# TensorSpeech/TensorFlowASR

Hardware: AMD Instinct MI355X
Metric: audio-hours/sec (train step) Conformer-M RNN-T (higher is better)
Workload: dtype bf16; 1 GPU; Conformer-M transducer full train step (fwd+RNN-T loss+bwd+Adam), LibriSpeech-shaped 16 kHz utterances, 32/GPU, padding=batch, SpecAugment on, dropout 0.1; global_batch=32, parallelism=dp1, params=32461288

## Files before the change

### include/tfasr_hip.h

```cpp
#ifndef TFASR_HIP_H_
#define TFASR_HIP_H_

#include <stddef.h>
#include <stdint.h>

#ifdef __cplusplus
extern "C" {
#endif

#define TFASR_ABI_VERSION 44

typedef enum {
  TFASR_STATUS_SUCCESS = 0,
  TFASR_STATUS_INVALID_VALUE = 1,
  TFASR_STATUS_EXECUTION_FAILED = 2,
  TFASR_STATUS_UNSUPPORTED = 3
} tfasr_status_t;

typedef enum { TFASR_F32 = 0, TFASR_BF16 = 1 } tfasr_dtype_t;

const char* tfasr_status_string(int status);
int tfasr_abi_version(void);
size_t tfasr_launch_count(void);

// ... 161 lines not shown

int tfasr_relattn_softmax_fwd(const void* content, const void* pos, const int32_t* lengths, void* probs, int B, int H,
                              int T, int ldc, int ldp, int use_mask, int dtype, void* stream);
int tfasr_relattn_softmax_bwd(const void* probs, const void* dprobs, const int32_t* lengths, void* dcontent, void* dpos,
                              int B, int H, int T, int ldc, int ldp, int use_mask, int dtype, void* stream);
int tfasr_relattn_softmax_fwd_streaming(const void* content, const void* pos, const int32_t* lengths, void* probs, int B, int H,
                                        int T, int ldc, int ldp, int use_mask, int chunk_size, int history_size, int dtype,
                                        void* stream);

int tfasr_relattn_fused_fwd(const void* qkv, const float* ubias, const float* vbias, const void* pext,
                            const int32_t* lengths, void* out, float* lse, int B, int H, int T, int dh, float scale,
                            int use_mask, int chunk, int hist, int dtype, void* stream);

int tfasr_relattn_fused_bwd_q3(const void* qkv, const float* ubias, const float* vbias, const void* pext, const int32_t* lengths,
                               const void* o, const void* dout, const float* lse, void* dq, long lddq, float* du, float* dv, void* ds,
                               float* dvec, float* dpext, void* qu, void* qv, int B, int H, int T, int dh, int lds, float scale, int use_mask,
                               int chunk, int hist, int dtype, void* stream);
int tfasr_relattn_dpext(const void* ds, const void* qv, const int32_t* lengths, float* dpext, int B, int H, int T, int dh, int lds,
                        int use_mask, int dtype, void* stream);
int tfasr_relattn_fused_bwd_k(const void* qkv, const void* qu, const void* qv, const void* pext, const int32_t* lengths,
                              const void* dout, const float* lse, const float* dvec, void* dqkv, int B, int H, int T, int dh,
                              float scale, int use_mask, int chunk, int hist, int dtype, void* stream);

int tfasr_lstm_step_fwd(const void* xg, long xg_stride_b, const float* hr, const void* h_prev, long hprev_stride_b,
                        const float* c_prev, long cprev_stride_b, const int32_t* lengths, int t, void* gates,
                        long gates_stride_b, float* c_out, long c_stride_b, void* h_out, long h_stride_b, void* y_out,
                        long y_stride_b, int B, int P, int dtype, void* stream);
int tfasr_lstm_step_bwd(const void* dy, long dy_stride_b, const float* dhr, float* dh_carry, float* dc_carry,
                        const void* gates, long gates_stride_b, const float* c_t, long c_stride_b, const float* c_prev,
                        long cprev_stride_b, const int32_t* lengths, int t, void* dz, long dz_stride_b, int B, int P,
                        int dtype, void* stream);

int tfasr_lstm_set_persist(int mode);
int tfasr_lstm_seq_fwd(const void* xg, const void* rk, const void* h0, long h0_stride_b, const float* c0, long c0_stride_b,
                       const int32_t* lengths, void* gates, float* cseq, void* hseq, void* yseq, float* hr, int B, int U1, int P,
                       int dtype, void* stream);
int tfasr_lstm_seq_bwd(const void* dy, const void* rk, const void* gates, const float* cseq, const int32_t* lengths, void* dz,
                       float* dh_carry, float* dc_carry, float* dhr, int B, int U1, int P, int dtype, void* stream);
int tfasr_lstm_seq_fwd_range(const void* xg, const void* rk, const void* h0, long h0_stride_b, const float* c0, long c0_stride_b,
                             const int32_t* lengths, void* gates, float* cseq, void* hseq, void* yseq, float* hr, int B, int U1, int P,
                             int dtype, int t0, int t1, void* stream);
int tfasr_lstm_seq_bwd_range(const void* dy, const void* rk, const void* gates, const float* cseq, const int32_t* lengths, void* dz,
                             float* dh_carry, float* dc_carry, float* dhr, int B, int U1, int P, int dtype, int t0, int t1, void* stream);
size_t tfasr_lstm_persist_sync_bytes(void);
int tfasr_lstm_persist_fwd(const void* xg, const void* rk, const void* h0, long h0_stride_b, const float* c0, long c0_stride_b,
                           const int32_t* lengths, void* gates, float* cseq, void* hseq, void* yseq, int B, int U1, int P, int dtype,
// ... 256 lines not shown
```

### tensorflowasr_amd/csrc/attn_fused.hip

```cpp
#include "common.h"
#ifdef TFASR_ATTN_TIMING
__device__ long long g_attn_timing[8 * 8192];
#define ATT_TICK(k) { const long long t_ = __builtin_readcyclecounter(); ph[k] += t_ - tp; tp = t_; }
#else
#define ATT_TICK(k)
#endif
#include <algorithm>
#include <stdlib.h>

typedef __attribute__((ext_vector_type(4))) short short4_t;

namespace {

#define LDS_PTR(p) ((__attribute__((address_space(3))) void*)(p))
#define GLB_PTR(p) ((const __attribute__((address_space(1))) void*)(p))

constexpr int DH = 64, BI = 64, BJ = 64, WIN = 128;
constexpr int SK_BYTES = BJ * DH * 2, SV_BYTES = BJ * DH * 2, SP_BYTES = WIN * DH * 2;
__device__ __forceinline__ int key_d(int row) { return (row & 3) | (((row >> 3) & 1) << 2); }
__device__ __forceinline__ int key_t64(int k) { return (((k >> 1) & 1) | (((k >> 3) & 1) << 1)) << 1; }

__device__ __forceinline__ void glds16_asm(const void* g, const char* lds_uniform) {
  const uint32_t l = (uint32_t)__builtin_amdgcn_readfirstlane((int)(uint32_t)(uintptr_t)lds_uniform);
  asm volatile("s_mov_b32 m0, %1\n\ts_nop 0\n\tglobal_load_lds_dwordx4 %0, off" ::"v"(g), "s"(l) : "memory");
// ... 46 lines not shown
  const int chunk = col >> 3, half = (col >> 2) & 1;
  const int k0 = kbase + (r >> 2), k1 = k0 + 4;
  const short4_t lo = __builtin_amdgcn_ds_read_tr16_b64_v4i16(
      (__attribute__((address_space(3))) short4_t*)(s + k0 * 128 + ((chunk ^ key_d(k0)) << 4) + half * 8));
  const short4_t hi = __builtin_amdgcn_ds_read_tr16_b64_v4i16(
      (__attribute__((address_space(3))) short4_t*)(s + k1 * 128 + ((chunk ^ key_d(k1)) << 4) + half * 8));
  short8_t v;
  v[0] = lo[0]; v[1] = lo[1]; v[2] = lo[2]; v[3] = lo[3];
  v[4] = hi[0]; v[5] = hi[1]; v[6] = hi[2]; v[7] = hi[3];
  return v;
}

__device__ __forceinline__ short8_t q_frag(const bf16_t* qrow, const float* bias, int k0) {
  float x[8];
  ld8(qrow + k0, x);
  short8_t f;
#pragma unroll
  for (int e = 0; e < 8; ++e) f[e] = (short)f32_to_bf16(x[e] + bias[k0 + e]);
  return f;
}

struct BlockId { int b, h, blk; bool ok; };
template <bool BLK_MAJOR = true>
__device__ __forceinline__ BlockId attn_block_id(int B, int H, int nblk) {
  const int lin = blockIdx.x, xcd = lin & 7, slot = lin >> 3;
  const int nbh = B * H, per = (nbh + 7) >> 3;
  const int blk = BLK_MAJOR ? slot / per : slot % nblk;
  const int bh = (BLK_MAJOR ? slot - blk * per : slot / nblk) * 8 + xcd;
  BlockId id;
  id.ok = bh < nbh && blk < nblk;
  id.b = bh / H; id.h = bh - id.b * H; id.blk = blk;
  return id;
}
inline unsigned attn_grid_size(int B, int H, int nblk) { return (unsigned)(8 * ((B * H + 7) / 8) * nblk); }

__device__ __forceinline__ void stream_window(int i, int T, int chunk, int hist, int& lo, int& hi) {
  const int index = (i / chunk) * chunk;
  lo = hist < 0 ? 0 : max(0, index - hist);
  hi = min(T, index + chunk);
}



constexpr int GLDT = 80, SGTT_BYTES = 16 * GLDT * 4 + 64;
__device__ __forceinline__ int strip_col(int il, int x) { return (((x >> 2) ^ ((il >> 1) & 3)) << 2) | (x & 3); }
constexpr int SMEM_FWDT = SK_BYTES + SV_BYTES + SP_BYTES + 4 * SGTT_BYTES;
static_assert((SMEM_FWDT + 1279) / 1280 * 3 <= 128, "three workgroups per CU");

template <bool STREAM>
__global__ __launch_bounds__(256, 3) void relattn_fused_fwdT_kernel(
    const bf16_t* __restrict__ qkv, const float* __restrict__ ubias, const float* __restrict__ vbias,
    const bf16_t* __restrict__ pext, const int32_t* __restrict__ lengths, bf16_t* __restrict__ out, float* __restrict__ lse_out,
    int B, int H, int T, float scale, int use_mask, int chunk, int hist) {
  extern __shared__ __attribute__((aligned(16))) char smem[];
  char* sK = smem;
  char* sV = sK + SK_BYTES;
// ... 223 lines not shown
#pragma unroll
    for (int n = 0; n < 4; ++n) {
      uint2 v;
      v.x = pack2_bf16(acc_o[n][0] * inv, acc_o[n][1] * inv);
      v.y = pack2_bf16(acc_o[n][2] * inv, acc_o[n][3] * inv);
      *reinterpret_cast<uint2*>(out + ((long)b * T + i) * HD + h * DH + n * 16 + g * 4) = v;
    }
    if (g == 0) lse_out[((long)b * H + h) * T + i] = m_run * 0.6931471805599453f + logf(l_run);
  }
}

constexpr int QT_IMG_LD = 272;
constexpr int QT_IMG_BYTES = 16 * QT_IMG_LD;
static_assert(QT_IMG_BYTES <= 16 * GLDT * 4, "the skewed dS image fits under the bias scores of the strip");
constexpr int qt_tile_bytes(int mode) { return (mode == 1 ? 2 : 1) * (SK_BYTES + SP_BYTES) + SV_BYTES; }
constexpr int qt_smem(int mode) { return qt_tile_bytes(mode) + 4 * SGTT_BYTES + (mode == 0 ? 4 * QT_IMG_BYTES : 0); }

__device__ __forceinline__ short8_t row_frag(const bf16_t* row, int k0) {
  return *reinterpret_cast<const short8_t*>(row + k0);
}

typedef float float2_t __attribute__((ext_vector_type(2)));

template <bool STREAM, int MODE>
__global__ __launch_bounds__(256, MODE == 2 ? 3 : 2) void relattn_fused_bwd_qT_kernel(
    const bf16_t* __restrict__ qkv, const float* __restrict__ ubias, const float* __restrict__ vbias,
    const bf16_t* __restrict__ pext, const int32_t* __restrict__ lengths, const bf16_t* __restrict__ o,
    const bf16_t* __restrict__ dout, const float* __restrict__ lse, bf16_t* __restrict__ dq, bf16_t* __restrict__ dpos,
    float* __restrict__ dvec, int B, int H, int T, int ldp, float scale, int use_mask, float* __restrict__ dpext,
    long lddq, float* __restrict__ du, float* __restrict__ dv, int chunk, int hist, bf16_t* qu_out, bf16_t* qv_out) {
  constexpr bool QT_PIPE = MODE == 1, QT_LEAN = MODE == 2, QT_ALIAS = MODE != 0;
  constexpr int QT_TILE_BYTES = qt_tile_bytes(MODE);
  extern __shared__ __attribute__((aligned(16))) char smem[];
  char* const sK0 = smem;
  char* const sV = sK0 + (QT_PIPE ? 2 : 1) * SK_BYTES;
  char* const sP0 = sV + SV_BYTES;
  char* const sStrips = smem + QT_TILE_BYTES;
  const int lane = threadIdx.x & 63, w = __builtin_amdgcn_readfirstlane(threadIdx.x >> 6);
  float* sG = reinterpret_cast<float*>(sStrips + w * SGTT_BYTES);
  float* sGb = sG + 16 * GLDT;
  char* sAg = QT_ALIAS ? reinterpret_cast<char*>(sG) : sStrips + 4 * SGTT_BYTES + w * QT_IMG_BYTES;
  const int r = lane & 15, g = lane >> 4;
  const BlockId bid = attn_block_id(B, H, (T + BI - 1) / BI);
  if (!bid.ok) return;
  const int b = bid.b, h = bid.h, i0 = bid.blk * BI;
  const int HD = H * DH, LDQ = 3 * HD, R = 2 * T - 1, R1 = 2 * T;
  const int len = lengths ? min(lengths[b], T) : T;
  const int shift = T - len;
  const bf16_t* qb = qkv + (long)b * T * LDQ + h * DH;
  const bf16_t* kb = qb + HD;
  const bf16_t* vb = qb + 2 * HD;
  const bf16_t* pb = pext + h * DH;
  uint4 bias_row = make_uint4(0, 0, 0, 0);
  if (MODE == 0 && (threadIdx.x >> 6) == 0 && (threadIdx.x & 63) < 8) bias_row = *reinterpret_cast<const uint4*>(pb + (long)(2 * T - 1) * HD + (((threadIdx.x & 63) ^ key_d(127)) << 3));

  const int i = i0 + w * 16 + r;
  if (use_mask && i0 >= len) {
    if (i < T) {
#pragma unroll
      for (int n = 0; n < 4; ++n) *reinterpret_cast<uint2*>(dq + ((long)b * T + i) * lddq + h * DH + n * 16 + g * 4) = make_uint2(0u, 0u);
    }
    return;
  }
  const int irow = min(i, T - 1);
  short8_t bqu[2], bqv[2], bdo[2];
  float dpart = 0.f;
#pragma unroll
  for (int kk = 0; kk < 2; ++kk) {
    bqu[kk] = q_frag(qb + (long)irow * LDQ, ubias + h * DH, kk * 32 + g * 8);
    bqv[kk] = q_frag(qb + (long)irow * LDQ, vbias + h * DH, kk * 32 + g * 8);
    const bf16_t* dorow = dout + ((long)b * T + irow) * HD + h * DH + kk * 32 + g * 8;
    const bf16_t* orow = o + ((long)b * T + irow) * HD + h * DH + kk * 32 + g * 8;
    bdo[kk] = row_frag(dorow, 0);
    float a[8], c[8];
    ld8(dorow, a);
    ld8(orow, c);
#pragma unroll
    for (int e = 0; e < 8; ++e) dpart += a[e] * c[e];
  }
  if (qu_out && i < T) {
#pragma unroll
    for (int kk = 0; kk < 2; ++kk) {
      *reinterpret_cast<short8_t*>(qu_out + ((long)b * T + irow) * HD + h * DH + kk * 32 + g * 8) = bqu[kk];
      *reinterpret_cast<short8_t*>(qv_out + ((long)b * T + irow) * HD + h * DH + kk * 32 + g * 8) = bqv[kk];
    }
  }
  dpart = xor32_sum(xor16_sum(dpart));
  if (g == 0 && i < T) dvec[((long)b * H + h) * T + i] = dpart;
  const float Di = dpart;
  const float scale2 = scale * 1.4426950408889634f;
  const float lse2 = lse[((long)b * H + h) * T + irow] * 1.4426950408889634f;
  const int lim = 2 * len - 1;
  const bool inrow = i < T;
  const bool live = inrow && !(use_mask && i >= len);
  const int jthr = lim - (T - 1 - i);
  int klo = 0, khi = T;
  if constexpr (STREAM) { if (live) stream_window(i, T, chunk, hist, klo, khi); }
  if (!live) khi = 0;
  int jl0[4], krow[4];
#pragma unroll
  for (int jt = 0; jt < 4; ++jt) {
    jl0[jt] = 32 * (jt >> 1) + g * 8 + (jt & 1) * 4;
    krow[jt] = 32 * (jt >> 1) + (r >> 2) * 8 + (jt & 1) * 4 + (r & 3);
  }
  int goff[4][4];
#pragma unroll
  for (int jt = 0; jt < 4; ++jt)
#pragma unroll
    for (int e = 0; e < 4; ++e) goff[jt][e] = r * GLDT + strip_col(r, 15 - r + jl0[jt] + e);
  char* const img = sAg + r * QT_IMG_LD + (63 - w * 16 - r + g * 8) * 2;
  float4_t acc_q[4], acc_v[4];
#pragma unroll
  for (int n = 0; n < 4; ++n) { acc_q[n] = float4_t{0.f, 0.f, 0.f, 0.f}; acc_v[n] = float4_t{0.f, 0.f, 0.f, 0.f}; }
  float bias_acc = 0.f;
  bf16_t* dsrow = dpos + (((long)b * H + h) * T + irow) * ldp;
  const int kk_lo = w < 2 ? 1 : 0;

  const int njb = (T + BJ - 1) / BJ;
  float gbias;
  if constexpr (QT_PIPE || QT_LEAN) {
    float part = 0.f;
#pragma unroll
    for (int kk = 0; kk < 2; ++kk) {
      float pr[8];
      ld8(pb + (long)R * HD + kk * 32 + g * 8, pr);
#pragma unroll
      for (int t = 0; t < 8; ++t) part += bf16_to_f32((bf16_t)bqv[kk][t]) * pr[t];
    }
    part = xor32_sum(xor16_sum(part));
    gbias = part;
  } else {
    char* const sP = sP0;
    if (w == 0 && lane < 8) *reinterpret_cast<uint4*>(sP + 127 * 128 + lane * 16) = bias_row;
    if constexpr (!QT_ALIAS) {
      const uint4 z4 = make_uint4(0, 0, 0, 0);
      for (int q = lane; q < QT_IMG_BYTES / 16; q += 64) *reinterpret_cast<uint4*>(sAg + q * 16) = z4;
    }
    __syncthreads();
    float4_t a = float4_t{0.f, 0.f, 0.f, 0.f};
#pragma unroll
    for (int kk = 0; kk < 2; ++kk) {
      short8_t f = frag_rows(sP, 112 + r, kk * 4 + g);
      if (r != 15) f = short8_t{0, 0, 0, 0, 0, 0, 0, 0};
      a = __builtin_amdgcn_mfma_f32_16x16x32_bf16(f, bqv[kk], a, 0, 0, 0);
    }
    if (g == 3) sGb[r] = a[3];
    asm volatile("s_waitcnt lgkmcnt(0)" ::: "memory");
    gbias = sGb[r];
  }
  if (g == 0 && i < T) dvec[(long)B * H * T + ((long)b * H + h) * T + i] = gbias;
  const float Dis = Di * scale;
  uint2 prb[4];
#pragma unroll
  for (int n = 0; n < 4; ++n) prb[n] = *reinterpret_cast<const uint2*>(pb + (long)R * HD + n * 16 + g * 4);
  const bf16_t* const fr_qu = qu_out + ((long)b * T + irow) * HD + h * DH + g * 8;
  const bf16_t* const fr_qv = qv_out + ((long)b * T + irow) * HD + h * DH + g * 8;
  const bf16_t* const fr_do = dout + ((long)b * T + irow) * HD + h * DH + g * 8;
  if constexpr (QT_LEAN) asm volatile("s_waitcnt vmcnt(0)" ::: "memory");
  if constexpr (QT_PIPE) {
    float l2 = lse2, gb = gbias, ds_ = Dis;
    asm volatile("" : "+v"(l2), "+v"(gb), "+v"(ds_));
    (void)l2; (void)gb; (void)ds_;
  }
#ifdef TFASR_ATTN_TIMING
  long long ph[5] = {0, 0, 0, 0, 0};
  const long long t_begin = __builtin_readcyclecounter();
#endif
  for (int jb = 0; jb < njb; ++jb) {
    const int j0 = jb * BJ;
    const int pw0 = (T - 1 - (i0 + BI - 1) + j0) + shift;
#ifdef TFASR_ATTN_TIMING
    long long tp = __builtin_readcyclecounter();
#endif
    char* sK = sK0;
    char* sP = sP0;
    if constexpr (QT_PIPE) {
      sK = sK0 + (jb & 1) * SK_BYTES;
      sP = sP0 + (jb & 1) * SP_BYTES;
      if (jb == 0) {
        load_rows<BJ, true>(sK, kb, LDQ, 0, T, w, lane);
        load_rows<BJ, true>(sV, vb, LDQ, 0, T, w, lane);
        load_rows<WIN, true>(sP, pb, HD, pw0, R1, w, lane);
      }
      asm volatile("s_waitcnt vmcnt(0)" ::: "memory");
      __builtin_amdgcn_s_barrier();
// ... 185 lines not shown
  for (int kk = 0; kk < 2; ++kk)
#pragma unroll
    for (int t = 0; t < 8; ++t) {
      float v = inrow ? bsum * bf16_to_f32((bf16_t)bqv[kk][t]) : 0.f;
      v = row16_sum(v);
      if (r == 0) red[(w * 3 + 2) * 64 + kk * 32 + g * 8 + t] = v;
    }
  __syncthreads();
  if (threadIdx.x < 192) {
    const int which = threadIdx.x >> 6, col = threadIdx.x & 63;
    const float v = red[(0 * 3 + which) * 64 + col] + red[(1 * 3 + which) * 64 + col] + red[(2 * 3 + which) * 64 + col] + red[(3 * 3 + which) * 64 + col];
    float* dst = which == 0 ? du + h * DH : which == 1 ? dv + h * DH : dpext + (long)R * HD + h * DH;
    if (which < 2 || v != 0.f) atomicAdd(dst + col, v);
  }
#ifdef TFASR_ATTN_TIMING
  if (threadIdx.x == 0 && blockIdx.x < 8192) {
    long long* o = g_attn_timing + 8L * blockIdx.x;
    for (int kq = 0; kq < 5; ++kq) o[kq] = ph[kq];
    o[5] = t_loop - t_begin; o[6] = __builtin_readcyclecounter() - t_loop; o[7] = njb;
  }
#endif
}


constexpr int DPX_TLD = 208;
constexpr int DPX_CHUNKS = 64 * (DPX_TLD / 8);
constexpr int DPX_TILE_BYTES = 7 * 256 * 16;
constexpr int DPX_BUF = DPX_TILE_BYTES + SK_BYTES;
constexpr int SMEM_DPX = 2 * DPX_BUF;

__global__ __launch_bounds__(256, 2) void relattn_dpext_kernel(
    const bf16_t* __restrict__ ds, const bf16_t* __restrict__ qv, const int32_t* __restrict__ lengths, float* __restrict__ dpext,
    int B, int H, int T, int lds, int use_mask, int bchunk) {
  extern __shared__ __attribute__((aligned(16))) char smem[];
  const int lane = threadIdx.x & 63, w = __builtin_amdgcn_readfirstlane(threadIdx.x >> 6);
  const int r = lane & 15, g = lane >> 4;
  const int c0 = blockIdx.x * 128, h = blockIdx.y;
  const int HD = H * DH, R = 2 * T - 1;
  const int b_lo = blockIdx.z * bchunk, b_hi = min(B, b_lo + bchunk);
  float4_t acc[2][4];
#pragma unroll
  for (int ct = 0; ct < 2; ++ct)
#pragma unroll
    for (int n = 0; n < 4; ++n) acc[ct][n] = float4_t{0.f, 0.f, 0.f, 0.f};
  const int nib = (T + BI - 1) / BI;

// ... 93 lines not shown
static_assert(K2_WAVE >= 4096, "the P^T and dS^T images fit over the strip slots");
constexpr int SMEM_BWD_K = 4 * SK_BYTES + SK_BYTES + SP_BYTES + 4 * K2_WAVE;
static_assert((SMEM_BWD_K + 1279) / 1280 * 2 <= 128, "two workgroups per CU");

__device__ __forceinline__ void img_store(char* s, int il, int g, float v0, float v1, float v2, float v3) {
  uint2 u;
  u.x = pack2_bf16(v0, v1);
  u.y = pack2_bf16(v2, v3);
  *reinterpret_cast<uint2*>(s + il * 32 + ((g ^ ((il >> 2) & 3)) << 3)) = u;
}
__device__ __forceinline__ short8_t img_frag(const char* s, int kbase, int r) {
  const int k0 = kbase + (r >> 2), k1 = k0 + 4, c = r & 3;
  const short4_t lo = __builtin_amdgcn_ds_read_tr16_b64_v4i16(
      (__attribute__((address_space(3))) short4_t*)(s + k0 * 32 + ((c ^ ((k0 >> 2) & 3)) << 3)));
  const short4_t hi = __builtin_amdgcn_ds_read_tr16_b64_v4i16(
      (__attribute__((address_space(3))) short4_t*)(s + k1 * 32 + ((c ^ ((k1 >> 2) & 3)) << 3)));
  short8_t v;
  v[0] = lo[0]; v[1] = lo[1]; v[2] = lo[2]; v[3] = lo[3];
  v[4] = hi[0]; v[5] = hi[1]; v[6] = hi[2]; v[7] = hi[3];
  return v;
}

template <bool STREAM>
__global__ __launch_bounds__(256, 2) void relattn_fused_bwd_k_kernel(
    const bf16_t* __restrict__ qkv, const bf16_t* __restrict__ qu, const bf16_t* __restrict__ qv,
    const bf16_t* __restrict__ pext, const int32_t* __restrict__ lengths, const bf16_t* __restrict__ dout,
    const float* __restrict__ lse, const float* __restrict__ dvec, bf16_t* __restrict__ dqkv, int B, int H, int T, float scale,
    int use_mask, int chunk, int hist) {
  extern __shared__ __attribute__((aligned(16))) char smem[];
  char* const sQu0 = smem;
  char* const sdO0 = sQu0 + 2 * SK_BYTES;
  char* const sQv = sdO0 + 2 * SK_BYTES;
  char* const sP = sQv + SK_BYTES;
  const int lane = threadIdx.x & 63, w = __builtin_amdgcn_readfirstlane(threadIdx.x >> 6);
  char* const sW = sP + SP_BYTES + w * K2_WAVE;
  float* const sS = reinterpret_cast<float*>(sW);
  char* const sAp = sW;
  char* const sAs = sW + 2048;
  const int r = lane & 15, g = lane >> 4;
  const BlockId bid = attn_block_id<false>(B, H, (T + BJ - 1) / BJ);
  if (!bid.ok) return;
  const int b = bid.b, h = bid.h, j0 = bid.blk * BJ;
  const int HD = H * DH, LDQ = 3 * HD, R1 = 2 * T;
  const int len = lengths ? min(lengths[b], T) : T;
  const int shift = T - len;
  const bf16_t* kb = qkv + (long)b * T * LDQ + HD + h * DH;
  const bf16_t* vb = kb + HD;
  const bf16_t* qub = qu + (long)b * T * HD + h * DH;
  const bf16_t* qvb = qv + (long)b * T * HD + h * DH;
  const bf16_t* dob = dout + (long)b * T * HD + h * DH;
  const bf16_t* pb = pext + h * DH;
  uint4 bias_row = make_uint4(0, 0, 0, 0);
  if ((threadIdx.x >> 6) == 0 && (threadIdx.x & 63) < 8) bias_row = *reinterpret_cast<const uint4*>(pb + (long)(2 * T - 1) * HD + (((threadIdx.x & 63) ^ key_d(127)) << 3));

  const int jrow = min(j0 + w * 16 + r, T - 1);
  short8_t ak[2], av[2];
#pragma unroll
  for (int kk = 0; kk < 2; ++kk) {
    ak[kk] = row_frag(kb + (long)jrow * LDQ, kk * 32 + g * 8);
    av[kk] = row_frag(vb + (long)jrow * LDQ, kk * 32 + g * 8);
  }
  float4_t acc_k[4], acc_v[4];
#pragma unroll
  for (int n = 0; n < 4; ++n) { acc_k[n] = float4_t{0.f, 0.f, 0.f, 0.f}; acc_v[n] = float4_t{0.f, 0.f, 0.f, 0.f}; }

// ... 177 lines not shown
#if defined(TFASR_ATTN_TIMING) && TFASR_ATTN_TIMING == 3
  if (threadIdx.x == 0 && blockIdx.x < 8192) {
    long long* o = g_attn_timing + 8L * blockIdx.x;
    for (int kq = 0; kq < 5; ++kq) o[kq] = ph[kq];
    o[5] = __builtin_readcyclecounter() - t_begin; o[6] = 0; o[7] = nfull;
  }
#endif
  {
    const int j = j0 + w * 16 + r;
    if (j < T) {
      bf16_t* row = dqkv + ((long)b * T + j) * LDQ + h * DH;
#pragma unroll
      for (int n = 0; n < 4; ++n) {
        uint2 vk, vv;
        vk.x = pack2_bf16(acc_k[n][0], acc_k[n][1]); vk.y = pack2_bf16(acc_k[n][2], acc_k[n][3]);
        vv.x = pack2_bf16(acc_v[n][0], acc_v[n][1]); vv.y = pack2_bf16(acc_v[n][2], acc_v[n][3]);
        *reinterpret_cast<uint2*>(row + HD + n * 16 + g * 4) = vk;
        *reinterpret_cast<uint2*>(row + 2 * HD + n * 16 + g * 4) = vv;
      }
    }
  }
}

}

extern "C" int tfasr_relattn_fused_fwd(const void* qkv, const float* ubias, const float* vbias, const void* pext,
                                       const int32_t* lengths, void* out, float* lse, int B, int H, int T, int dh, float scale,
                                       int use_mask, int chunk, int hist, int dtype, void* stream_) {
  if (!qkv || !ubias || !vbias || !pext || !out || !lse || B <= 0 || H <= 0 || T <= 0) return TFASR_STATUS_INVALID_VALUE;
  if (dtype != TFASR_BF16 || dh != DH) return TFASR_STATUS_UNSUPPORTED;
  const dim3 gridT(attn_grid_size(B, H, (T + BI - 1) / BI));
  if (chunk > 0) TFASR_KLAUNCH(relattn_fused_fwdT_kernel<true>, gridT, dim3(256), SMEM_FWDT, (hipStream_t)stream_, (const bf16_t*)qkv, ubias, vbias,
                                    (const bf16_t*)pext, lengths, (bf16_t*)out, lse, B, H, T, scale, use_mask, chunk, hist);
  else TFASR_KLAUNCH(relattn_fused_fwdT_kernel<false>, gridT, dim3(256), SMEM_FWDT, (hipStream_t)stream_, (const bf16_t*)qkv, ubias, vbias,
                          (const bf16_t*)pext, lengths, (bf16_t*)out, lse, B, H, T, scale, use_mask, chunk, hist);
  TFASR_CHECK_LAUNCH();
  return TFASR_STATUS_SUCCESS;
}

extern "C" int tfasr_relattn_fused_bwd_q3(const void* qkv, const float* ubias, const float* vbias, const void* pext, const int32_t* lengths,
                                          const void* o, const void* dout, const float* lse, void* dq, long lddq, float* du, float* dv, void* ds,
                                          float* dvec, float* dpext, void* qu, void* qv, int B, int H, int T, int dh, int lds, float scale,
                                          int use_mask, int chunk, int hist, int dtype, void* stream_) {
  if (!qkv || !ubias || !vbias || !pext || !o || !dout || !lse || !dq || !du || !dv || !ds || !dvec || !dpext || B <= 0 || H <= 0 || T <= 0 || lds < T ||
      (lds & 7) || lddq < (long)H * dh || (lddq & 3) || ((qu == nullptr) != (qv == nullptr)) || (((uintptr_t)qu | (uintptr_t)qv) & 15))
    return TFASR_STATUS_INVALID_VALUE;
// ... 31 lines not shown
}

extern "C" int tfasr_relattn_fused_bwd_k(const void* qkv, const void* qu, const void* qv, const void* pext, const int32_t* lengths,
                                         const void* dout, const float* lse, const float* dvec, void* dqkv, int B, int H, int T,
                                         int dh, float scale, int use_mask, int chunk, int hist, int dtype, void* stream_) {
  if (!qkv || !qu || !qv || !pext || !dout || !lse || !dvec || !dqkv || B <= 0 || H <= 0 || T <= 0) return TFASR_STATUS_INVALID_VALUE;
  if (dtype != TFASR_BF16 || dh != DH) return TFASR_STATUS_UNSUPPORTED;
  const dim3 gk(attn_grid_size(B, H, (T + BJ - 1) / BJ));
  static bool attr_done = false;
  if (!attr_done) {
    (void)hipFuncSetAttribute((const void*)relattn_fused_bwd_k_kernel<true>, hipFuncAttributeMaxDynamicSharedMemorySize, SMEM_BWD_K);
    (void)hipFuncSetAttribute((const void*)relattn_fused_bwd_k_kernel<false>, hipFuncAttributeMaxDynamicSharedMemorySize, SMEM_BWD_K);
    attr_done = true;
  }
#define TFASR_BK_LAUNCH(KERN, SMEM, ST, CH, HI)                                                                                         \
  TFASR_KLAUNCH((KERN<ST>), gk, dim3(256), SMEM, (hipStream_t)stream_, (const bf16_t*)qkv, (const bf16_t*)qu, (const bf16_t*)qv,        \
                (const bf16_t*)pext, lengths, (const bf16_t*)dout, lse, dvec, (bf16_t*)dqkv, B, H, T, scale, use_mask, CH, HI)
  if (chunk > 0) TFASR_BK_LAUNCH(relattn_fused_bwd_k_kernel, SMEM_BWD_K, true, chunk, hist); else TFASR_BK_LAUNCH(relattn_fused_bwd_k_kernel, SMEM_BWD_K, false, 0, 0);
#undef TFASR_BK_LAUNCH
  TFASR_CHECK_LAUNCH();
  return TFASR_STATUS_SUCCESS;
}

#ifdef TFASR_ATTN_TIMING
extern "C" int tfasr_attn_timing_read(long long* out, int n) {
  if (hipDeviceSynchronize() != hipSuccess) return 1;
  return hipMemcpyFromSymbol(out, HIP_SYMBOL(g_attn_timing), sizeof(long long) * n) == hipSuccess ? 0 : 1;
}
#endif
```

### tensorflowasr_amd/csrc/block.hip

```cpp
#include "common.h"
#include <string.h>
#include <stdlib.h>
#include <vector>

extern int g_tfasr_group_beside;

bool tfasr_bn_rows_kernel_ok(int C);
namespace {

struct Arena {
  char* base;
  size_t off, cap;
  bool ok;
  size_t peak;
  void* get(size_t n) {
    const size_t a = (off + 255) & ~(size_t)255;
    if (base && a + n > cap) { ok = false; return nullptr; }
    off = a + n;
    if (off > peak) peak = off;
    return base ? base + a : (void*)(uintptr_t)256;
  }
};

struct Ctx {
// ... 364 lines not shown
      gemm(g);
    }
    void* dqkv = act(scratch, rows * 3 * HD);
    bool dq_done = false;
    void* dqu = act(scratch, rows * HD);
    void* dqv = act(scratch, rows * HD);
    const bool v2 = k->fused;
    void* dpos = act(scratch, v2 ? (long)B * H * T * Tp : (long)B * H * T * R1p);
    const bool dpext_deferred = !dry && v2 && io->defer_pos_grad && io->dpext_zero && io->ds_keep && io->qv_keep;
    if (dpext_deferred) dpos = io->ds_keep;
    if (!dry && dpext_deferred) k->left |= 1;
    const void* qv;
    float tail_scale;
    float* dpext = io->dpext_zero;
    if (v2) {
      if (!dpext) {
        dpext = f32(scratch, (long)R1 * HD);
        zero(dpext, (size_t)R1 * HD * 4);
      }
      float* dvec = f32(scratch, 2L * B * H * T);
      void* qu = act(scratch, rows * HD);
      void* qvb = act(scratch, rows * HD);
      if (dpext_deferred) qvb = io->qv_keep;
      if (!dry) {
        chk(tfasr_relattn_fused_bwd_q3(k->at_qkv, fp(TFASR_BP_AT_U), fp(TFASR_BP_AT_V), k->at_pext, io->lengths, k->at_att, datt, k->at_lse, dqkv,
                                       3L * HD, gp(TFASR_BP_AT_U), gp(TFASR_BP_AT_V), dpos, dvec, dpext, qu, qvb, B, H, T, dh, Tp, scale, c->use_mask,
                                       c->chunk_size, c->history_size, c->dtype, s));
        dq_done = true;
        chk(tfasr_relattn_fused_bwd_k(k->at_qkv, qu, qvb, k->at_pext, io->lengths, datt, k->at_lse, dvec, dqkv, B, H, T, dh, scale, c->use_mask,
                                      c->chunk_size, c->history_size, c->dtype, s));
        if (!dpext_deferred) chk(tfasr_relattn_dpext(dpos, qvb, io->lengths, dpext, B, H, T, dh, Tp, c->use_mask, c->dtype, s));
      }
      qv = qvb;
      tail_scale = 1.f;
    } else {
      const char* kk = (const char*)k->at_qkv + (size_t)HD * esz;
      const char* vv = (const char*)k->at_qkv + (size_t)2 * HD * esz;
      char* dk = (char*)dqkv + (size_t)HD * esz;
      char* dv = (char*)dqkv + (size_t)2 * HD * esz;
      void* dprobs = act(scratch, (long)B * H * T * Tp);
      G a; a.A = datt; a.lda = HD; a.ta = 0; a.B = vv; a.ldb = 3 * HD; a.tb = 1; a.D = dprobs; a.ldd = Tp; a.M = T; a.N = T; a.K = dh;
      a.nb1 = B; a.nb2 = H; a.sA1 = (long)T * HD; a.sA2 = dh; a.sB1 = (long)T * 3 * HD; a.sB2 = dh; a.sD1 = (long)H * T * Tp; a.sD2 = (long)T * Tp;
      gemm(a);
      G b; b.A = k->at_probs; b.lda = Tp; b.ta = 1; b.B = datt; b.ldb = HD; b.tb = 0; b.D = dv; b.ldd = 3 * HD; b.M = T; b.N = dh; b.K = T;
      b.nb1 = B; b.nb2 = H; b.sA1 = (long)H * T * Tp; b.sA2 = (long)T * Tp; b.sB1 = (long)T * HD; b.sB2 = dh; b.sD1 = (long)T * 3 * HD; b.sD2 = dh;
      gemm(b);
      if (!dry) chk(tfasr_relattn_softmax_bwd(k->at_probs, dprobs, io->lengths, dprobs, dpos, B, H, T, Tp, R1p, c->use_mask, c->dtype, s));
// ... 424 lines not shown
```

### tensorflowasr_amd/kernels.py

```python
import ctypes
import os

import torch

from . import _lib
from ._lib import ACT_FACTOR, ACT_NONE, ACT_SIGMOID, ACT_SWISH, ACT_TANH, ACT_TANH_OUT, TFASR_BF16, TFASR_F32, GemmArgs, check

_WS_CACHE = {}
_SPLITK_WS = False


def _dt(t):
    if t.dtype == torch.float32:
        return TFASR_F32
    if t.dtype == torch.bfloat16:
        return TFASR_BF16
    raise TypeError(f"unsupported activation dtype {t.dtype}")


def _p(t):
    if t is None:
        return None
    if not t.is_cuda:
        raise _lib.TfasrError("tensorflowasr_amd ops need HIP device tensors (no CPU fallback on the product path)")
# ... 678 lines not shown
    if ds is None:
        ds = torch.empty(B, H, T, lds, dtype=qkv.dtype, device=qkv.device)
    dvec = torch.empty(2, B, H, T, dtype=torch.float32, device=qkv.device)
    qu = torch.empty(B * T, H * dh, dtype=qkv.dtype, device=qkv.device)
    if qv is None:
        qv = torch.empty(B * T, H * dh, dtype=qkv.dtype, device=qkv.device)
    check(_L().tfasr_relattn_fused_bwd_q3(_p(qkv), _p(ubias), _p(vbias), _p(pext), _p(lengths), _p(o), _p(dout), _p(lse), _p(dqkv), dqkv.stride(0),
                                          _p(du), _p(dv), _p(ds), _p(dvec), _p(dpext), _p(qu), _p(qv), B, H, T, dh, lds, scale, int(use_mask),
                                          *_window(chunk_size, history_size), _dt(qkv), _stream()), "relattn_fused_bwd_q3")
    return ds, dvec, qu, qv


def relattn_dpext(ds, qv, lengths, dpext, B, H, T, dh, use_mask=True):
    check(_L().tfasr_relattn_dpext(_p(ds), _p(qv), _p(lengths), _p(dpext), B, H, T, dh, ds.shape[3], int(use_mask), _dt(ds), _stream()), "relattn_dpext")
    return dpext


def relattn_fused_bwd_k(qkv, qu, qv, pext, lengths, dout, lse, dvec, dqkv, B, H, T, dh, scale, use_mask=True, chunk_size=None, history_size=None):
    check(_L().tfasr_relattn_fused_bwd_k(_p(qkv), _p(qu), _p(qv), _p(pext), _p(lengths), _p(dout), _p(lse), _p(dvec), _p(dqkv), B, H, T, dh,
                                         scale, int(use_mask), *_window(chunk_size, history_size), _dt(qkv), _stream()), "relattn_fused_bwd_k")
    return dqkv


def lstm_step_fwd(xg_t, hr, h_prev, c_prev, lengths, t, gates_t, c_out, h_out, y_out, B, P):
    check(_L().tfasr_lstm_step_fwd(
        _pv(xg_t), xg_t.stride(0), _pv(hr), _pv(h_prev), 0 if h_prev is None else h_prev.stride(0), _pv(c_prev),
        0 if c_prev is None else c_prev.stride(0), _pv(lengths), t, _pv(gates_t), 0 if gates_t is None else gates_t.stride(0),
        _pv(c_out), c_out.stride(0), _pv(h_out), h_out.stride(0), _pv(y_out), 0 if y_out is None else y_out.stride(0), B, P,
        _dt(xg_t), _stream()), "lstm_step_fwd")


def lstm_step_bwd(dy_t, dhr, dh_carry, dc_carry, gates_t, c_t, c_prev, lengths, t, dz_t, B, P):
    check(_L().tfasr_lstm_step_bwd(
        _pv(dy_t), dy_t.stride(0), _pv(dhr), _pv(dh_carry), _pv(dc_carry), _pv(gates_t), gates_t.stride(0), _pv(c_t), c_t.stride(0),
        _pv(c_prev), 0 if c_prev is None else c_prev.stride(0), _pv(lengths), t, _pv(dz_t), dz_t.stride(0), B, P, _dt(dy_t),
        _stream()), "lstm_step_bwd")


def lstm_set_persist(mode):
    return int(_L().tfasr_lstm_set_persist(int(mode)))


def lstm_seq_fwd(xg, rk, h0, c0, lengths, gates, cseq, hseq, yseq, hr):
    B, U1, P4 = xg.shape
    P = P4 // 4
    assert xg.is_contiguous() and gates.is_contiguous() and cseq.is_contiguous() and hseq.is_contiguous() and (yseq is None or yseq.is_contiguous())
# ... 870 lines not shown
```

Measured before the change: 4.745 audio-hours/sec.

## Merge attention backward dQ and dK/dV kernels into one launch with prep pass

Measured after the change: 4.816 audio-hours/sec, median of 6. 1.01x the previous value.

```diff
diff --git a/include/tfasr_hip.h b/include/tfasr_hip.h
--- a/include/tfasr_hip.h
+++ b/include/tfasr_hip.h
@@ -207,6 +207,14 @@
                               const void* dout, const float* lse, const float* dvec, void* dqkv, int B, int H, int T, int dh,
                               float scale, int use_mask, int chunk, int hist, int dtype, void* stream);
 
+int tfasr_relattn_bwd_prep(const void* qkv, const float* ubias, const float* vbias, const void* pext, const int32_t* lengths,
+                           const void* o, const void* dout, void* qu, void* qv, float* dvec, int32_t* order, int B, int H, int T,
+                           int dh, int use_mask, int dtype, void* stream);
+int tfasr_relattn_fused_bwd_qk(const void* qkv, const float* ubias, const float* vbias, const void* pext, const int32_t* lengths,
+                               const void* dout, const float* lse, const void* qu, const void* qv, const float* dvec,
+                               const int32_t* order, void* dqkv, float* du, float* dv, void* ds, float* dpext, int B, int H, int T, int dh,
+                               int lds, float scale, int use_mask, int chunk, int hist, int dtype, void* stream);
+
 int tfasr_lstm_step_fwd(const void* xg, long xg_stride_b, const float* hr, const void* h_prev, long hprev_stride_b,
                         const float* c_prev, long cprev_stride_b, const int32_t* lengths, int t, void* gates,
                         long gates_stride_b, float* c_out, long c_stride_b, void* h_out, long h_stride_b, void* y_out,
diff --git a/tensorflowasr_amd/csrc/attn_fused.hip b/tensorflowasr_amd/csrc/attn_fused.hip
--- a/tensorflowasr_amd/csrc/attn_fused.hip
+++ b/tensorflowasr_amd/csrc/attn_fused.hip
@@ -92,8 +92,8 @@
 
 struct BlockId { int b, h, blk; bool ok; };
 template <bool BLK_MAJOR = true>
-__device__ __forceinline__ BlockId attn_block_id(int B, int H, int nblk) {
-  const int lin = blockIdx.x, xcd = lin & 7, slot = lin >> 3;
+__device__ __forceinline__ BlockId attn_block_id(int B, int H, int nblk, int lin) {
+  const int xcd = lin & 7, slot = lin >> 3;
   const int nbh = B * H, per = (nbh + 7) >> 3;
   const int blk = BLK_MAJOR ? slot / per : slot % nblk;
   const int bh = (BLK_MAJOR ? slot - blk * per : slot / nblk) * 8 + xcd;
@@ -102,6 +102,8 @@
   id.b = bh / H; id.h = bh - id.b * H; id.blk = blk;
   return id;
 }
+template <bool BLK_MAJOR = true>
+__device__ __forceinline__ BlockId attn_block_id(int B, int H, int nblk) { return attn_block_id<BLK_MAJOR>(B, H, nblk, (int)blockIdx.x); }
 inline unsigned attn_grid_size(int B, int H, int nblk) { return (unsigned)(8 * ((B * H + 7) / 8) * nblk); }
 
 __device__ __forceinline__ void stream_window(int i, int T, int chunk, int hist, int& lo, int& hi) {
@@ -371,8 +373,37 @@
 
 typedef float float2_t __attribute__((ext_vector_type(2)));
 
-template <bool STREAM, int MODE>
-__global__ __launch_bounds__(256, MODE == 2 ? 3 : 2) void relattn_fused_bwd_qT_kernel(
+__device__ __forceinline__ float qrow_frags(const bf16_t* qrow, const float* ub, const float* vb, const bf16_t* dorow, const bf16_t* orow, int g,
+                                            short8_t (&bqu)[2], short8_t (&bqv)[2], short8_t (&bdo)[2]) {
+  float dpart = 0.f;
+#pragma unroll
+  for (int kk = 0; kk < 2; ++kk) {
+    bqu[kk] = q_frag(qrow, ub, kk * 32 + g * 8);
+    bqv[kk] = q_frag(qrow, vb, kk * 32 + g * 8);
+    bdo[kk] = row_frag(dorow + kk * 32 + g * 8, 0);
+    float a[8], c[8];
+    ld8(dorow + kk * 32 + g * 8, a);
+    ld8(orow + kk * 32 + g * 8, c);
+#pragma unroll
+    for (int e = 0; e < 8; ++e) dpart += a[e] * c[e];
+  }
+  return dpart;
+}
+__device__ __forceinline__ float qrow_bias_part(const short8_t (&bqv)[2], const bf16_t* prow, int g) {
+  float part = 0.f;
+#pragma unroll
+  for (int kk = 0; kk < 2; ++kk) {
+    float pr[8];
+    ld8(prow + kk * 32 + g * 8, pr);
+#pragma unroll
+    for (int t = 0; t < 8; ++t) part += bf16_to_f32((bf16_t)bqv[kk][t]) * pr[t];
+  }
+  return part;
+}
+
+template <bool STREAM, int MODE, bool PRE>
+__device__ __forceinline__ void relattn_bwd_qT_body(
+    char* const smem, const int lin,
     const bf16_t* __restrict__ qkv, const float* __restrict__ ubias, const float* __restrict__ vbias,
     const bf16_t* __restrict__ pext, const int32_t* __restrict__ lengths, const bf16_t* __restrict__ o,
     const bf16_t* __restrict__ dout, const float* __restrict__ lse, bf16_t* __restrict__ dq, bf16_t* __restrict__ dpos,
@@ -380,7 +411,7 @@
     long lddq, float* __restrict__ du, float* __restrict__ dv, int chunk, int hist, bf16_t* qu_out, bf16_t* qv_out) {
   constexpr bool QT_PIPE = MODE == 1, QT_LEAN = MODE == 2, QT_ALIAS = MODE != 0;
   constexpr int QT_TILE_BYTES = qt_tile_bytes(MODE);
-  extern __shared__ __attribute__((aligned(16))) char smem[];
+  static_assert(!PRE || MODE == 1, "the reading mode exists for the pipelined build only");
   char* const sK0 = smem;
   char* const sV = sK0 + (QT_PIPE ? 2 : 1) * SK_BYTES;
   char* const sP0 = sV + SV_BYTES;
@@ -390,7 +421,7 @@
   float* sGb = sG + 16 * GLDT;
   char* sAg = QT_ALIAS ? reinterpret_cast<char*>(sG) : sStrips + 4 * SGTT_BYTES + w * QT_IMG_BYTES;
   const int r = lane & 15, g = lane >> 4;
-  const BlockId bid = attn_block_id(B, H, (T + BI - 1) / BI);
+  const BlockId bid = attn_block_id(B, H, (T + BI - 1) / BI, lin);
   if (!bid.ok) return;
   const int b = bid.b, h = bid.h, i0 = bid.blk * BI;
   const int HD = H * DH, LDQ = 3 * HD, R = 2 * T - 1, R1 = 2 * T;
@@ -414,28 +445,30 @@
   const int irow = min(i, T - 1);
   short8_t bqu[2], bqv[2], bdo[2];
   float dpart = 0.f;
-#pragma unroll
-  for (int kk = 0; kk < 2; ++kk) {
-    bqu[kk] = q_frag(qb + (long)irow * LDQ, ubias + h * DH, kk * 32 + g * 8);
-    bqv[kk] = q_frag(qb + (long)irow * LDQ, vbias + h * DH, kk * 32 + g * 8);
-    const bf16_t* dorow = dout + ((long)b * T + irow) * HD + h * DH + kk * 32 + g * 8;
-    const bf16_t* orow = o + ((long)b * T + irow) * HD + h * DH + kk * 32 + g * 8;
-    bdo[kk] = row_frag(dorow, 0);
-    float a[8], c[8];
-    ld8(dorow, a);
-    ld8(orow, c);
-#pragma unroll
-    for (int e = 0; e < 8; ++e) dpart += a[e] * c[e];
-  }
-  if (qu_out && i < T) {
+  if constexpr (PRE) {
+#pragma unroll
+    for (int kk = 0; kk < 2; ++kk) {
+      bqu[kk] = row_frag(qu_out + ((long)b * T + irow) * HD + h * DH, kk * 32 + g * 8);
+      bqv[kk] = row_frag(qv_out + ((long)b * T + irow) * HD + h * DH, kk * 32 + g * 8);
+      bdo[kk] = row_frag(dout + ((long)b * T + irow) * HD + h * DH, kk * 32 + g * 8);
+    }
+  } else {
+    dpart = qrow_frags(qb + (long)irow * LDQ, ubias + h * DH, vbias + h * DH, dout + ((long)b * T + irow) * HD + h * DH,
+                       o + ((long)b * T + irow) * HD + h * DH, g, bqu, bqv, bdo);
+  }
+  if (!PRE && qu_out && i < T) {
 #pragma unroll
     for (int kk = 0; kk < 2; ++kk) {
       *reinterpret_cast<short8_t*>(qu_out + ((long)b * T + irow) * HD + h * DH + kk * 32 + g * 8) = bqu[kk];
       *reinterpret_cast<short8_t*>(qv_out + ((long)b * T + irow) * HD + h * DH + kk * 32 + g * 8) = bqv[kk];
     }
   }
-  dpart = xor32_sum(xor16_sum(dpart));
-  if (g == 0 && i < T) dvec[((long)b * H + h) * T + i] = dpart;
+  if constexpr (PRE) {
+    dpart = dvec[((long)b * H + h) * T + irow];
+  } else {
+    dpart = xor32_sum(xor16_sum(dpart));
+    if (g == 0 && i < T) dvec[((long)b * H + h) * T + i] = dpart;
+  }
   const float Di = dpart;
   const float scale2 = scale * 1.4426950408889634f;
   const float lse2 = lse[((long)b * H + h) * T + irow] * 1.4426950408889634f;
@@ -467,17 +500,10 @@
 
   const int njb = (T + BJ - 1) / BJ;
   float gbias;
-  if constexpr (QT_PIPE || QT_LEAN) {
-    float part = 0.f;
-#pragma unroll
-    for (int kk = 0; kk < 2; ++kk) {
-      float pr[8];
-      ld8(pb + (long)R * HD + kk * 32 + g * 8, pr);
-#pragma unroll
-      for (int t = 0; t < 8; ++t) part += bf16_to_f32((bf16_t)bqv[kk][t]) * pr[t];
-    }
-    part = xor32_sum(xor16_sum(part));
-    gbias = part;
+  if constexpr (PRE) {
+    gbias = dvec[(long)B * H * T + ((long)b * H + h) * T + irow];
+  } else if constexpr (QT_PIPE || QT_LEAN) {
+    gbias = xor32_sum(xor16_sum(qrow_bias_part(bqv, pb + (long)R * HD, g)));
   } else {
     char* const sP = sP0;
     if (w == 0 && lane < 8) *reinterpret_cast<uint4*>(sP + 127 * 128 + lane * 16) = bias_row;
@@ -497,7 +523,7 @@
     asm volatile("s_waitcnt lgkmcnt(0)" ::: "memory");
     gbias = sGb[r];
   }
-  if (g == 0 && i < T) dvec[(long)B * H * T + ((long)b * H + h) * T + i] = gbias;
+  if (!PRE && g == 0 && i < T) dvec[(long)B * H * T + ((long)b * H + h) * T + i] = gbias;
   const float Dis = Di * scale;
   uint2 prb[4];
 #pragma unroll
@@ -510,6 +536,10 @@
     float l2 = lse2, gb = gbias, ds_ = Dis;
     asm volatile("" : "+v"(l2), "+v"(gb), "+v"(ds_));
     (void)l2; (void)gb; (void)ds_;
+    if constexpr (PRE) {
+#pragma unroll
+      for (int kk = 0; kk < 2; ++kk) asm volatile("" : "+v"(bqu[kk]), "+v"(bqv[kk]), "+v"(bdo[kk]));
+    }
   }
 #ifdef TFASR_ATTN_TIMING
   long long ph[5] = {0, 0, 0, 0, 0};
@@ -741,6 +771,18 @@
 #endif
 }
 
+template <bool STREAM, int MODE>
+__global__ __launch_bounds__(256, MODE == 2 ? 3 : 2) void relattn_fused_bwd_qT_kernel(
+    const bf16_t* __restrict__ qkv, const float* __restrict__ ubias, const float* __restrict__ vbias,
+    const bf16_t* __restrict__ pext, const int32_t* __restrict__ lengths, const bf16_t* __restrict__ o,
+    const bf16_t* __restrict__ dout, const float* __restrict__ lse, bf16_t* __restrict__ dq, bf16_t* __restrict__ dpos,
+    float* __restrict__ dvec, int B, int H, int T, int ldp, float scale, int use_mask, float* __restrict__ dpext,
+    long lddq, float* __restrict__ du, float* __restrict__ dv, int chunk, int hist, bf16_t* qu_out, bf16_t* qv_out) {
+  extern __shared__ __attribute__((aligned(16))) char smem[];
+  relattn_bwd_qT_body<STREAM, MODE, false>(smem, (int)blockIdx.x, qkv, ubias, vbias, pext, lengths, o, dout, lse, dq, dpos, dvec, B, H, T, ldp, scale,
+                                           use_mask, dpext, lddq, du, dv, chunk, hist, qu_out, qv_out);
+}
+
 
 constexpr int DPX_TLD = 208;
 constexpr int DPX_CHUNKS = 64 * (DPX_TLD / 8);
@@ -880,12 +922,12 @@
 }
 
 template <bool STREAM>
-__global__ __launch_bounds__(256, 2) void relattn_fused_bwd_k_kernel(
+__device__ __forceinline__ void relattn_bwd_k_body(
+    char* const smem, const int lin, const int32_t* __restrict__ order,
     const bf16_t* __restrict__ qkv, const bf16_t* __restrict__ qu, const bf16_t* __restrict__ qv,
     const bf16_t* __restrict__ pext, const int32_t* __restrict__ lengths, const bf16_t* __restrict__ dout,
     const float* __restrict__ lse, const float* __restrict__ dvec, bf16_t* __restrict__ dqkv, int B, int H, int T, float scale,
     int use_mask, int chunk, int hist) {
-  extern __shared__ __attribute__((aligned(16))) char smem[];
   char* const sQu0 = smem;
   char* const sdO0 = sQu0 + 2 * SK_BYTES;
   char* const sQv = sdO0 + 2 * SK_BYTES;
@@ -896,9 +938,9 @@
   char* const sAp = sW;
   char* const sAs = sW + 2048;
   const int r = lane & 15, g = lane >> 4;
-  const BlockId bid = attn_block_id<false>(B, H, (T + BJ - 1) / BJ);
+  const BlockId bid = attn_block_id<false>(B, H, (T + BJ - 1) / BJ, lin);
   if (!bid.ok) return;
-  const int b = bid.b, h = bid.h, j0 = bid.blk * BJ;
+  const int b = order ? order[bid.b] : bid.b, h = bid.h, j0 = bid.blk * BJ;
   const int HD = H * DH, LDQ = 3 * HD, R1 = 2 * T;
   const int len = lengths ? min(lengths[b], T) : T;
   const int shift = T - len;
@@ -1122,6 +1164,77 @@
   }
 }
 
+template <bool STREAM>
+__global__ __launch_bounds__(256, 2) void relattn_fused_bwd_k_kernel(
+    const bf16_t* __restrict__ qkv, const bf16_t* __restrict__ qu, const bf16_t* __restrict__ qv,
+    const bf16_t* __restrict__ pext, const int32_t* __restrict__ lengths, const bf16_t* __restrict__ dout,
+    const float* __restrict__ lse, const float* __restrict__ dvec, bf16_t* __restrict__ dqkv, int B, int H, int T, float scale,
+    int use_mask, int chunk, int hist) {
+  extern __shared__ __attribute__((aligned(16))) char smem[];
+  relattn_bwd_k_body<STREAM>(smem, (int)blockIdx.x, nullptr, qkv, qu, qv, pext, lengths, dout, lse, dvec, dqkv, B, H, T, scale, use_mask, chunk, hist);
+}
+
+constexpr int SMEM_BWD_QK = qt_smem(1) > SMEM_BWD_K ? qt_smem(1) : SMEM_BWD_K;
+static_assert((SMEM_BWD_QK + 1279) / 1280 * 2 <= 128, "two workgroups per CU");
+
+template <bool STREAM>
+__global__ __launch_bounds__(256, 2) void relattn_fused_bwd_qk_kernel(
+    const bf16_t* __restrict__ qkv, const float* __restrict__ ubias, const float* __restrict__ vbias, const bf16_t* __restrict__ pext,
+    const int32_t* __restrict__ lengths, const bf16_t* __restrict__ dout, const float* __restrict__ lse, const bf16_t* __restrict__ qu,
+    const bf16_t* __restrict__ qv, const float* __restrict__ dvec, const int32_t* __restrict__ order, bf16_t* __restrict__ dqkv,
+    bf16_t* __restrict__ dpos, float* __restrict__ dpext, float* __restrict__ du, float* __restrict__ dv, int B, int H, int T, int ldp,
+    float scale, int use_mask, int chunk, int hist, int nq) {
+  extern __shared__ __attribute__((aligned(16))) char smem[];
+  const int lin = (int)blockIdx.x;
+  if (lin < nq) {
+    relattn_bwd_qT_body<STREAM, 1, true>(smem, lin, qkv, ubias, vbias, pext, lengths, nullptr, dout, lse, dqkv, dpos, const_cast<float*>(dvec), B, H, T,
+                                         ldp, scale, use_mask, dpext, 3L * H * DH, du, dv, chunk, hist, const_cast<bf16_t*>(qu), const_cast<bf16_t*>(qv));
+  } else {
+    relattn_bwd_k_body<STREAM>(smem, lin - nq, order, qkv, qu, qv, pext, lengths, dout, lse, dvec, dqkv, B, H, T, scale, use_mask, chunk, hist);
+  }
+}
+
+__global__ __launch_bounds__(256) void relattn_bwd_prep_kernel(
+    const bf16_t* __restrict__ qkv, const float* __restrict__ ubias, const float* __restrict__ vbias, const bf16_t* __restrict__ pext,
+    const int32_t* __restrict__ lengths, const bf16_t* __restrict__ o, const bf16_t* __restrict__ dout, bf16_t* __restrict__ qu_out,
+    bf16_t* __restrict__ qv_out, float* __restrict__ dvec, int32_t* __restrict__ order, int B, int H, int T, int use_mask) {
+  if (blockIdx.x == 0 && blockIdx.y == 0 && blockIdx.z == 0) {
+    for (int s = threadIdx.x; s < B; s += 256) {
+      const int ls = lengths ? min(lengths[s], T) : T;
+      int rank = 0;
+      for (int t = 0; t < B; ++t) {
+        const int lt = lengths ? min(lengths[t], T) : T;
+        rank += (lt > ls || (lt == ls && t < s)) ? 1 : 0;
+      }
+      order[rank] = s;
+    }
+  }
+  const int lane = threadIdx.x & 63, w = threadIdx.x >> 6;
+  const int r = lane & 15, g = lane >> 4;
+  const int b = blockIdx.z, h = blockIdx.y, i0 = blockIdx.x * BI;
+  const int HD = H * DH, LDQ = 3 * HD, R = 2 * T - 1;
+  const int len = lengths ? min(lengths[b], T) : T;
+  if (use_mask && i0 >= len) return;
+  const int i = i0 + w * 16 + r;
+  const int irow = min(i, T - 1);
+  const long orow = ((long)b * T + irow) * HD + h * DH;
+  short8_t bqu[2], bqv[2], bdo[2];
+  float dpart = qrow_frags(qkv + ((long)b * T + irow) * LDQ + h * DH, ubias + h * DH, vbias + h * DH, dout + orow, o + orow, g, bqu, bqv, bdo);
+  dpart = xor32_sum(xor16_sum(dpart));
+  const float gbias = xor32_sum(xor16_sum(qrow_bias_part(bqv, pext + (long)R * HD + h * DH, g)));
+  if (i < T) {
+#pragma unroll
+    for (int kk = 0; kk < 2; ++kk) {
+      *reinterpret_cast<short8_t*>(qu_out + orow + kk * 32 + g * 8) = bqu[kk];
+      *reinterpret_cast<short8_t*>(qv_out + orow + kk * 32 + g * 8) = bqv[kk];
+    }
+    if (g == 0) {
+      dvec[((long)b * H + h) * T + i] = dpart;
+      dvec[(long)B * H * T + ((long)b * H + h) * T + i] = gbias;
+    }
+  }
+}
+
 }
 
 extern "C" int tfasr_relattn_fused_fwd(const void* qkv, const float* ubias, const float* vbias, const void* pext,
@@ -1199,6 +1312,44 @@
   return TFASR_STATUS_SUCCESS;
 }
 
+extern "C" int tfasr_relattn_bwd_prep(const void* qkv, const float* ubias, const float* vbias, const void* pext, const int32_t* lengths,
+                                      const void* o, const void* dout, void* qu, void* qv, float* dvec, int32_t* order, int B, int H, int T,
+                                      int dh, int use_mask, int dtype, void* stream_) {
+  if (!qkv || !ubias || !vbias || !pext || !o || !dout || !qu || !qv || !dvec || !order || B <= 0 || H <= 0 || T <= 0 || B > 65535 || H > 65535 ||
+      (((uintptr_t)qu | (uintptr_t)qv) & 15))
+    return TFASR_STATUS_INVALID_VALUE;
+  if (dtype != TFASR_BF16 || dh != DH) return TFASR_STATUS_UNSUPPORTED;
+  TFASR_KLAUNCH(relattn_bwd_prep_kernel, dim3((T + BI - 1) / BI, H, B), dim3(256), 0, (hipStream_t)stream_, (const bf16_t*)qkv, ubias, vbias,
+                (const bf16_t*)pext, lengths, (const bf16_t*)o, (const bf16_t*)dout, (bf16_t*)qu, (bf16_t*)qv, dvec, order, B, H, T, use_mask);
+  TFASR_CHECK_LAUNCH();
+  return TFASR_STATUS_SUCCESS;
+}
+
+extern "C" int tfasr_relattn_fused_bwd_qk(const void* qkv, const float* ubias, const float* vbias, const void* pext, const int32_t* lengths,
+                                          const void* dout, const float* lse, const void* qu, const void* qv, const float* dvec,
+                                          const int32_t* order, void* dqkv, float* du, float* dv, void* ds, float* dpext, int B, int H, int T, int dh,
+                                          int lds, float scale, int use_mask, int chunk, int hist, int dtype, void* stream_) {
+  if (!qkv || !ubias || !vbias || !pext || !dout || !lse || !qu || !qv || !dvec || !order || !dqkv || !du || !dv || !ds || !dpext || B <= 0 || H <= 0 ||
+      T <= 0 || lds < T || (lds & 7) || (((uintptr_t)qu | (uintptr_t)qv) & 15))
+    return TFASR_STATUS_INVALID_VALUE;
+  if (dtype != TFASR_BF16 || dh != DH) return TFASR_STATUS_UNSUPPORTED;
+  static bool attr_done = false;
+  if (!attr_done) {
+    (void)hipFuncSetAttribute((const void*)relattn_fused_bwd_qk_kernel<true>, hipFuncAttributeMaxDynamicSharedMemorySize, SMEM_BWD_QK);
+    (void)hipFuncSetAttribute((const void*)relattn_fused_bwd_qk_kernel<false>, hipFuncAttributeMaxDynamicSharedMemorySize, SMEM_BWD_QK);
+    attr_done = true;
+  }
+  const unsigned nq = attn_grid_size(B, H, (T + BI - 1) / BI), nk = attn_grid_size(B, H, (T + BJ - 1) / BJ);
+#define TFASR_QK_LAUNCH(ST, CH, HI)                                                                                                          \
+  TFASR_KLAUNCH((relattn_fused_bwd_qk_kernel<ST>), dim3(nq + nk), dim3(256), SMEM_BWD_QK, (hipStream_t)stream_, (const bf16_t*)qkv, ubias, vbias, \
+                (const bf16_t*)pext, lengths, (const bf16_t*)dout, lse, (const bf16_t*)qu, (const bf16_t*)qv, dvec, order, (bf16_t*)dqkv,   \
+                (bf16_t*)ds, dpext, du, dv, B, H, T, lds, scale, use_mask, CH, HI, (int)nq)
+  if (chunk > 0) TFASR_QK_LAUNCH(true, chunk, hist); else TFASR_QK_LAUNCH(false, 0, 0);
+#undef TFASR_QK_LAUNCH
+  TFASR_CHECK_LAUNCH();
+  return TFASR_STATUS_SUCCESS;
+}
+
 #ifdef TFASR_ATTN_TIMING
 extern "C" int tfasr_attn_timing_read(long long* out, int n) {
   if (hipDeviceSynchronize() != hipSuccess) return 1;
diff --git a/tensorflowasr_amd/csrc/block.hip b/tensorflowasr_amd/csrc/block.hip
--- a/tensorflowasr_amd/csrc/block.hip
+++ b/tensorflowasr_amd/csrc/block.hip
@@ -410,7 +410,18 @@
       void* qu = act(scratch, rows * HD);
       void* qvb = act(scratch, rows * HD);
       if (dpext_deferred) qvb = io->qv_keep;
-      if (!dry) {
+      int32_t* order = (int32_t*)f32(scratch, B);
+      const char* qk_env = getenv("TFASR_ATTN_BWD_QK");
+      const bool merged = qk_env ? qk_env[0] != '0' : true;
+      if (!dry && merged) {
+        chk(tfasr_relattn_bwd_prep(k->at_qkv, fp(TFASR_BP_AT_U), fp(TFASR_BP_AT_V), k->at_pext, io->lengths, k->at_att, datt, qu, qvb, dvec, order,
+                                   B, H, T, dh, c->use_mask, c->dtype, s));
+        chk(tfasr_relattn_fused_bwd_qk(k->at_qkv, fp(TFASR_BP_AT_U), fp(TFASR_BP_AT_V), k->at_pext, io->lengths, datt, k->at_lse, qu, qvb, dvec, order,
+                                       dqkv, gp(TFASR_BP_AT_U), gp(TFASR_BP_AT_V), dpos, dpext, B, H, T, dh, Tp, scale, c->use_mask,
+                                       c->chunk_size, c->history_size, c->dtype, s));
+        dq_done = true;
+        if (!dpext_deferred) chk(tfasr_relattn_dpext(dpos, qvb, io->lengths, dpext, B, H, T, dh, Tp, c->use_mask, c->dtype, s));
+      } else if (!dry) {
         chk(tfasr_relattn_fused_bwd_q3(k->at_qkv, fp(TFASR_BP_AT_U), fp(TFASR_BP_AT_V), k->at_pext, io->lengths, k->at_att, datt, k->at_lse, dqkv,
                                        3L * HD, gp(TFASR_BP_AT_U), gp(TFASR_BP_AT_V), dpos, dvec, dpext, qu, qvb, B, H, T, dh, Tp, scale, c->use_mask,
                                        c->chunk_size, c->history_size, c->dtype, s));
diff --git a/tensorflowasr_amd/kernels.py b/tensorflowasr_amd/kernels.py
--- a/tensorflowasr_amd/kernels.py
+++ b/tensorflowasr_amd/kernels.py
@@ -724,6 +724,30 @@
     return dqkv
 
 
+def relattn_bwd_prep(qkv, ubias, vbias, pext, lengths, o, dout, B, H, T, dh, use_mask=True, qu=None, qv=None, dvec=None):
+    if qu is None:
+        qu = torch.empty(B * T, H * dh, dtype=qkv.dtype, device=qkv.device)
+    if qv is None:
+        qv = torch.empty(B * T, H * dh, dtype=qkv.dtype, device=qkv.device)
+    if dvec is None:
+        dvec = torch.empty(2, B, H, T, dtype=torch.float32, device=qkv.device)
+    order = torch.empty(B, dtype=torch.int32, device=qkv.device)
+    check(_L().tfasr_relattn_bwd_prep(_p(qkv), _p(ubias), _p(vbias), _p(pext), _p(lengths), _p(o), _p(dout), _p(qu), _p(qv), _p(dvec), _p(order),
+                                      B, H, T, dh, int(use_mask), _dt(qkv), _stream()), "relattn_bwd_prep")
+    return qu, qv, dvec, order
+
+
+def relattn_fused_bwd_qk(qkv, ubias, vbias, pext, lengths, dout, lse, qu, qv, dvec, order, dqkv, du, dv, dpext, B, H, T, dh, scale, use_mask=True,
+                         chunk_size=None, history_size=None, ds=None):
+    lds = -(-T // 8) * 8
+    if ds is None:
+        ds = torch.empty(B, H, T, lds, dtype=qkv.dtype, device=qkv.device)
+    check(_L().tfasr_relattn_fused_bwd_qk(_p(qkv), _p(ubias), _p(vbias), _p(pext), _p(lengths), _p(dout), _p(lse), _p(qu), _p(qv), _p(dvec),
+                                          _p(order), _p(dqkv), _p(du), _p(dv), _p(ds), _p(dpext), B, H, T, dh, lds, scale, int(use_mask),
+                                          *_window(chunk_size, history_size), _dt(qkv), _stream()), "relattn_fused_bwd_qk")
+    return ds
+
+
 def lstm_step_fwd(xg_t, hr, h_prev, c_prev, lengths, t, gates_t, c_out, h_out, y_out, B, P):
     check(_L().tfasr_lstm_step_fwd(
         _pv(xg_t), xg_t.stride(0), _pv(hr), _pv(h_prev), 0 if h_prev is None else h_prev.stride(0), _pv(c_prev),
```
